# monkey0head/RePlay_cql

Measured on AMD Instinct MI355X. Metric: CQL train-steps/sec, higher is better.
Workload: dtype bf16; 1 GPU; BASELINE.json configs[2]: synthetic 1000000 users x 100000 items, CQL d=128, L=50, B=4096/GPU, bf16 MFMA + fp32 accumulate; users=1000000, items=100000, d=128, window=50, batch_per_gpu=4096, global_batch=4096, parallelism=dp1 (users sharded by rank, RCCL gradient all-reduce), k=10, dp_variant=single

## Files before the change

replay_cql_amd/csrc/common.h:

```cpp
#pragma once
#include <hip/hip_runtime.h>
#include <stdint.h>
#include <stdio.h>
#include <stdarg.h>

#include "../../include/cqlrec.h"

typedef __attribute__((ext_vector_type(8))) __bf16 bf16x8;
typedef __attribute__((ext_vector_type(4))) __bf16 bf16x4;
typedef __attribute__((ext_vector_type(16))) float f32x16;
typedef __attribute__((ext_vector_type(4))) float f32x4;
typedef __attribute__((address_space(3))) bf16x4 lds_bf16x4;

#define CQL_WAVE 64
#define CQL_LOG2E 1.4426950408889634f
#define CQL_LN2 0.6931471805599453f
#define NEG_INF_F (-__builtin_inff())

void cql_set_error(const char* fmt, ...);
#define CQL_REQUIRE(cond, ...)            \
  do {                                    \
    if (!(cond)) {                        \
      cql_set_error(__VA_ARGS__);         \
      return CQLREC_ERR_INVALID;          \
// ... 59 lines not shown
}

__device__ __forceinline__ int mfma_row(int reg, int half) { return (reg & 3) + 8 * (reg >> 2) + 4 * half; }

template <int D>
__device__ __forceinline__ int swz_chunk(int row, int ch) {
  if constexpr (D == 64) return ch ^ ((row >> 1) & 7);
  else return ch ^ (row & 15);
}

__device__ __forceinline__ float fast_exp2(float x) { return __builtin_amdgcn_exp2f(x); }

__device__ __forceinline__ uint32_t f32_order_key(float f) {
  uint32_t u = __float_as_uint(f);
  return (u & 0x80000000u) ? ~u : (u | 0x80000000u);
}
__device__ __forceinline__ float f32_from_order_key(uint32_t k) {
  uint32_t u = (k & 0x80000000u) ? (k & 0x7FFFFFFFu) : ~k;
  return __uint_as_float(u);
}

struct CqlAdamFix {
  int valid;
  const float* slab;
  const float* slab_cs;
  int32_t G, T, nblk, items, D;
  float scale;
  int64_t n_items;
  int64_t rows_off, cs_off;
};
int cql_adam_ema_fix(float* theta, float* grads, float* m, float* v, float* target, uint16_t* theta_b, uint16_t* target_b,
                     int64_t n, float step_size, float sqrt_bc2, float beta1, float beta2, float eps, float tau,
                     int32_t zero_grads, const CqlAdamFix* fix, hipStream_t stream);
int cql_adam_ema_rows(float* theta, float* grads, float* m, float* v, float* target, uint16_t* theta_b, uint16_t* target_b,
                      int64_t n, float step_size, float sqrt_bc2, float beta1, float beta2, float eps, float tau,
                      int32_t zero_grads, const uint8_t* row_map, int32_t d, int64_t n_rows, hipStream_t stream);
int cql_gather_pool_bwd_mark_rows(const void* ws, int64_t n_states, int32_t L, int32_t d, int64_t n_items, uint8_t* row_map,
                                  hipStream_t s);
```

replay_cql_amd/csrc/gbwd.hip:

```cpp
#include <cstring>
#include <rocprim/device/device_radix_sort.hpp>

#include "common.h"

__global__ __launch_bounds__(256) void gbwd_pairs_kernel(const int64_t* __restrict__ offsets,
                                                         const int32_t* __restrict__ items,
                                                         const int32_t* __restrict__ users,
                                                         const int32_t* __restrict__ ends, int end_delta,
                                                         int64_t n_states, int L, uint32_t pad_key,
                                                         uint32_t* __restrict__ keys, uint32_t* __restrict__ vals,
                                                         int32_t* __restrict__ lens) {
  const int lane = threadIdx.x & 63;
  const int64_t state = (int64_t)blockIdx.x * 4 + (threadIdx.x >> 6);
  if (state >= n_states) return;
  const int u = users[state];
  const int64_t o0 = offsets[u];
  const int end = ends ? (ends[state] + end_delta) : (int)(offsets[u + 1] - o0);
  const int len = end < L ? end : L;
  if (lane == 0) lens[state] = len;
  const int32_t* win = items + o0 + end - len;
  for (int j = lane; j < L; j += 64) {
    keys[state * L + j] = (j < len) ? (uint32_t)win[j] : pad_key;
    vals[state * L + j] = (uint32_t)state;
  }
// ... 200 lines not shown
  if (e != hipSuccess) {
    cql_set_error("gather_pool_bwd_prepare: radix sort failed: %s", hipGetErrorString(e));
    return CQLREC_ERR_HIP;
  }
  CQL_LAUNCH_CHECK("gather_pool_bwd_prepare");
  return CQLREC_OK;
}

__global__ __launch_bounds__(256) void gbwd_mark_rows_kernel(const uint32_t* __restrict__ keys, int64_t n_pairs,
                                                             uint32_t pad_key, uint8_t* __restrict__ row_map) {
  const int64_t i = (int64_t)blockIdx.x * blockDim.x + threadIdx.x;
  if (i >= n_pairs) return;
  const uint32_t k = keys[i];
  if (k < pad_key) row_map[k] = 1;
}
int cql_gather_pool_bwd_mark_rows(const void* ws, int64_t n_states, int32_t L, int32_t d, int64_t n_items, uint8_t* row_map,
                                  hipStream_t s) {
  CQL_REQUIRE(ws && row_map, "gather_pool_bwd_mark_rows: NULL pointer");
  CQL_REQUIRE(n_items > 0 && n_items < (1ll << 31), "gather_pool_bwd_mark_rows: n_items=%lld", (long long)n_items);
  if (hipMemsetAsync(row_map, 0, (size_t)n_items, s) != hipSuccess) {
    cql_set_error("gather_pool_bwd_mark_rows: clearing the map failed");
    return CQLREC_ERR_HIP;
  }
  if (n_states <= 0) return CQLREC_OK;
  const GbWs w = gb_carve(const_cast<void*>(ws), n_states, L, d);
  const int64_t n = n_states * L;
  CqlProfScope prof(CQLREC_PH_GATHER_BWD, s);
  hipLaunchKernelGGL(gbwd_mark_rows_kernel, dim3(cql_ceil_div(n, 256)), dim3(256), 0, s, w.keys_out, n, (uint32_t)n_items,
                     row_map);
  CQL_LAUNCH_CHECK("gather_pool_bwd_mark_rows");
  return CQLREC_OK;
}

extern "C" int cqlrec_gather_pool_bwd_apply(const float* dh0, int64_t n_states, int32_t L, int32_t d, int64_t n_items,
                                            void* ws, int64_t ws_bytes, float* g_E_in, cqlrec_stream stream) {
  CQL_REQUIRE(dh0 && ws && g_E_in, "gather_pool_bwd_apply: NULL pointer");
  CQL_REQUIRE(d == 64 || d == 128 || d == 256, "gather_pool_bwd_apply: d=%d unsupported", d);
  if (n_states <= 0) return CQLREC_OK;
  CQL_REQUIRE(ws_bytes >= cqlrec_gather_pool_bwd_ws_bytes(n_states, L, d), "gather_pool_bwd_apply: workspace too small");
  const GbWs w = gb_carve(ws, n_states, L, d);
  const int64_t n = n_states * L;
  hipStream_t s = (hipStream_t)stream;
  const uint32_t pad_key = (uint32_t)n_items;
  CqlProfScope prof(CQLREC_PH_GATHER_BWD, s);
  const int64_t n4 = n_states * (d / 4);
  hipLaunchKernelGGL(gbwd_scale_kernel, dim3(cql_ceil_div(n4, 256)), dim3(256), 0, s, (const float4*)dh0, w.lens, n4,
                     d / 4, (float4*)w.g);
  segsum_launch<false, GB_CH>(w.g, nullptr, w.keys_out, w.vals_out, n, pad_key, d, g_E_in, nullptr, w.edge, nullptr, s);
  CQL_LAUNCH_CHECK("gather_pool_bwd_apply");
  return CQLREC_OK;
}

extern "C" int cqlrec_gather_pool_bwd_sorted(const float* dh0, const int64_t* offsets, const int32_t* items,
                                             const int32_t* users, const int32_t* ends, int32_t end_delta,
                                             int64_t n_states, int32_t L, int32_t d, int64_t n_items, void* ws,
                                             int64_t ws_bytes, float* g_E_in, cqlrec_stream stream) {
  int rc = cqlrec_gather_pool_bwd_prepare(offsets, items, users, ends, end_delta, n_states, L, d, n_items, ws, ws_bytes,
                                          stream);
  if (rc != CQLREC_OK) return rc;
  return cqlrec_gather_pool_bwd_apply(dh0, n_states, L, d, n_items, ws, ws_bytes, g_E_in, stream);
}


namespace {
struct OhWs {
  uint32_t *keys_in, *vals_in, *keys_out, *vals_out;
// ... 65 lines not shown
```

replay_cql_amd/csrc/misc.hip:

```cpp
#include <stdlib.h>
#include "common.h"
#include "adam_math.h"

static thread_local char g_err[512] = "";
void cql_set_error(const char* fmt, ...) {
  va_list ap;
  va_start(ap, fmt);
  vsnprintf(g_err, sizeof(g_err), fmt, ap);
  va_end(ap);
}
extern "C" const char* cqlrec_last_error(void) { return g_err; }
extern "C" int cqlrec_abi_version(void) { return CQLREC_ABI_VERSION; }

#define CQL_PROF_POOL 8192
static struct {
  bool on = false;
  bool created = false;
  hipEvent_t ev[CQL_PROF_POOL][2];
  int phase[CQL_PROF_POOL];
  int n = 0;
  int open = -1;
  uint32_t mask = 0xFFFFFFFFu;
} g_prof;

// ... 661 lines not shown
  CQL_LAUNCH_CHECK("td_loss");
  return CQLREC_OK;
}

template <bool NT>
__global__ __launch_bounds__(256) void adam_ema_kernel(float4* __restrict__ theta, float4* __restrict__ grads,
                                                       float4* __restrict__ m, float4* __restrict__ v,
                                                       float4* __restrict__ target, uint2* __restrict__ theta_b,
                                                       uint2* __restrict__ target_b, int64_t n4, float step_size,
                                                       float sqrt_bc2, float beta1, float beta2, float eps, float tau,
                                                       int zero_grads) {
  const float omb1 = 1.0f - beta1, omb2 = 1.0f - beta2, omt = 1.0f - tau;
  for (int64_t i = (int64_t)blockIdx.x * blockDim.x + threadIdx.x; i < n4; i += (int64_t)gridDim.x * blockDim.x) {
    const float4 g4 = ld4<NT>(grads + i);
    float4 p4 = ld4<NT>(theta + i), m4 = ld4<NT>(m + i), v4 = ld4<NT>(v + i), t4 = ld4<NT>(target + i);
    const float g[4] = {g4.x, g4.y, g4.z, g4.w};
    float p[4] = {p4.x, p4.y, p4.z, p4.w}, mm[4] = {m4.x, m4.y, m4.z, m4.w}, vv[4] = {v4.x, v4.y, v4.z, v4.w},
          tt[4] = {t4.x, t4.y, t4.z, t4.w};
#pragma unroll
    for (int k = 0; k < 4; ++k) {
      adam_ema_elem(g[k], p[k], mm[k], vv[k], tt[k], step_size, sqrt_bc2, beta1, beta2, eps, tau, omb1, omb2, omt);
    }
    st4<NT>(theta + i, p[0], p[1], p[2], p[3]);
    st4<NT>(m + i, mm[0], mm[1], mm[2], mm[3]);
    st4<NT>(v + i, vv[0], vv[1], vv[2], vv[3]);
    st4<NT>(target + i, tt[0], tt[1], tt[2], tt[3]);
    theta_b[i] = make_uint2(pack_bf16x2(p[0], p[1]), pack_bf16x2(p[2], p[3]));
    target_b[i] = make_uint2(pack_bf16x2(tt[0], tt[1]), pack_bf16x2(tt[2], tt[3]));
    if (zero_grads) st4<NT>(grads + i, 0.f, 0.f, 0.f, 0.f);
  }
}

template <bool NT>
__global__ __launch_bounds__(256) void adam_ema_rows_kernel(float4* __restrict__ theta, float4* __restrict__ grads,
                                                            float4* __restrict__ m, float4* __restrict__ v,
                                                            float4* __restrict__ target, uint2* __restrict__ theta_b,
                                                            uint2* __restrict__ target_b, int64_t n4, float step_size,
                                                            float sqrt_bc2, float beta1, float beta2, float eps, float tau,
                                                            int zero_grads, const uint8_t* __restrict__ row_map, int ld4row,
                                                            int64_t n_rows) {
  const float omb1 = 1.0f - beta1, omb2 = 1.0f - beta2, omt = 1.0f - tau;
  for (int64_t i = (int64_t)blockIdx.x * blockDim.x + threadIdx.x; i < n4; i += (int64_t)gridDim.x * blockDim.x) {
    const int64_t row = i >> ld4row;
    const bool live = row < n_rows && row_map[row] != 0;
    float4 p4 = ld4<NT>(theta + i), m4 = ld4<NT>(m + i), v4 = ld4<NT>(v + i), t4 = ld4<NT>(target + i);
    float4 g4 = make_float4(0.f, 0.f, 0.f, 0.f);
    if (live) g4 = ld4<NT>(grads + i);
    const float g[4] = {g4.x, g4.y, g4.z, g4.w};
    float p[4] = {p4.x, p4.y, p4.z, p4.w}, mm[4] = {m4.x, m4.y, m4.z, m4.w}, vv[4] = {v4.x, v4.y, v4.z, v4.w},
          tt[4] = {t4.x, t4.y, t4.z, t4.w};
#pragma unroll
    for (int k = 0; k < 4; ++k) {
      adam_ema_elem(g[k], p[k], mm[k], vv[k], tt[k], step_size, sqrt_bc2, beta1, beta2, eps, tau, omb1, omb2, omt);
    }
    st4<NT>(theta + i, p[0], p[1], p[2], p[3]);
    st4<NT>(m + i, mm[0], mm[1], mm[2], mm[3]);
    st4<NT>(v + i, vv[0], vv[1], vv[2], vv[3]);
    st4<NT>(target + i, tt[0], tt[1], tt[2], tt[3]);
    theta_b[i] = make_uint2(pack_bf16x2(p[0], p[1]), pack_bf16x2(p[2], p[3]));
    target_b[i] = make_uint2(pack_bf16x2(tt[0], tt[1]), pack_bf16x2(tt[2], tt[3]));
    if (zero_grads) st4<NT>(grads + i, 0.f, 0.f, 0.f, 0.f);
  }
}

int cql_adam_ema_rows(float* theta, float* grads, float* m, float* v, float* target, uint16_t* theta_b, uint16_t* target_b,
                      int64_t n, float step_size, float sqrt_bc2, float beta1, float beta2, float eps, float tau,
                      int32_t zero_grads, const uint8_t* row_map, int32_t d, int64_t n_rows, hipStream_t stream) {
  CQL_REQUIRE(theta && grads && m && v && target && theta_b && target_b && row_map, "adam_ema_rows: NULL pointer");
  CQL_REQUIRE(n > 0 && n % 4 == 0, "adam_ema_rows: n=%lld must be a positive multiple of 4", (long long)n);
  CQL_REQUIRE(d == 64 || d == 128 || d == 256, "adam_ema_rows: d=%d unsupported", d);
  CQL_REQUIRE(n_rows >= 0 && n_rows * d <= n, "adam_ema_rows: %lld rows of %d do not fit n=%lld", (long long)n_rows, d,
              (long long)n);
  const int64_t n4 = n / 4;
  int blocks = (int)((n4 + 255) / 256);
  if (blocks > 8192) blocks = 8192;
  CqlProfScope prof(CQLREC_PH_ADAM, stream);
  hipLaunchKernelGGL(adam_ema_rows_kernel<true>, dim3(blocks), dim3(256), 0, stream, (float4*)theta, (float4*)grads,
                     (float4*)m, (float4*)v, (float4*)target, (uint2*)theta_b, (uint2*)target_b, n4, step_size, sqrt_bc2,
                     beta1, beta2, eps, tau, zero_grads, row_map, __builtin_ctz((unsigned)d) - 2, n_rows);
  CQL_LAUNCH_CHECK("adam_ema (row map)");
  return CQLREC_OK;
}

__device__ __forceinline__ void adam_fix4(const CqlAdamFix& f, float (&g)[4], int64_t i4, int ld, int li) {
  const int64_t e = 4 * i4;
  uint32_t item;
  int col = -1;
  if (e >= f.rows_off && e < f.rows_off + f.n_items * f.D) {
    const uint64_t r = (uint64_t)(e - f.rows_off);
    item = (uint32_t)(r >> ld);
    col = (int)(r & (uint64_t)(f.D - 1));
  } else if (e >= f.cs_off && e < f.cs_off + f.n_items) {
    item = (uint32_t)(e - f.cs_off);
  } else {
    return;
  }
#ifdef ADAMFIX_ABL_NOLOOP
  return;
#endif
  const uint32_t grp = item >> li, row = item & (uint32_t)(f.items - 1);
  const uint32_t W = (uint32_t)f.G * (uint32_t)f.T, nblk = (uint32_t)f.nblk, lo = grp * (uint32_t)f.T, hi = lo + (uint32_t)f.T;
  for (uint32_t p = ((lo + 1) * nblk + W - 1) / W; p < nblk; ++p) {
    const uint32_t u0 = (uint32_t)((uint64_t)p * W / nblk);
    if (u0 >= hi) break;
    if (u0 <= lo) continue;
    if ((uint32_t)(((uint64_t)p + 1) * W / nblk) == u0) continue;
    if (col >= 0) {
      const float4 s4 = *reinterpret_cast<const float4*>(f.slab + ((int64_t)p * f.items + row) * f.D + col);
      g[0] += f.scale * s4.x; g[1] += f.scale * s4.y; g[2] += f.scale * s4.z; g[3] += f.scale * s4.w;
    } else {
      const float* sc = f.slab_cs + (int64_t)p * f.items + row;
#pragma unroll
      for (int k = 0; k < 4; ++k)
// ... 93 lines not shown
```

replay_cql_amd/csrc/train.hip:

```cpp
#include <math.h>
#include <stdlib.h>
#include "common.h"
#include "qhead_internal.h"

static int g_concurrency = -1;

enum { MK_LOSS = 0, MK_DH, MK_DE, MK_CHAIN, MK_ADAM_IN, MK_ADAM_OUT, MK_PROLOGUE, MK_LSE, MK_NEXT_LOSS, MK_ENC_DX, MK_GATHER_BWD, MK_SORT_NEXT, MK_COUNT };
static hipEvent_t g_marks[MK_COUNT];
static int g_marks_on = 0;
static int g_mark_phase = 0;
static void mark(int k, hipStream_t s) {
  if (g_marks_on && g_mark_phase) (void)hipEventRecord(g_marks[k], s);
}
extern "C" int cqlrec_debug_marks_enable(int32_t on) {
  if (on && !g_marks[0])
    for (int i = 0; i < MK_COUNT; ++i)
      if (hipEventCreate(&g_marks[i]) != hipSuccess) return CQLREC_ERR_HIP;
  g_marks_on = on ? 1 : 0;
  return CQLREC_OK;
}
extern "C" int cqlrec_debug_marks_read(float* ms_out) {
  if (!g_marks[0] || !ms_out) return CQLREC_ERR_INVALID;
  for (int i = 0; i < MK_COUNT; ++i) {
    ms_out[i] = -1.f;
    if (hipEventSynchronize(g_marks[i]) != hipSuccess) continue;
    float ms = 0.f;
    if (hipEventElapsedTime(&ms, g_marks[MK_LOSS], g_marks[i]) == hipSuccess) ms_out[i] = ms;
  }
  return CQLREC_OK;
}

namespace {
struct Carve {
  char* base;
  int64_t off;
  explicit Carve(void* p) : base((char*)p), off(0) {}
  template <typename T>
  T* take(int64_t n) {
    T* p = base ? (T*)(base + off) : nullptr;
    off += (n * (int64_t)sizeof(T) + 255) / 256 * 256;
    return p;
  }
};

struct StepWs {
  int32_t *users, *tpos, *act, *a_star;
  float *rew, *done, *q_a, *lse, *nlse2, *nlse_nat, *q_targ, *y, *coef, *maxv, *loss, *term;
  float *h0_s, *dH, *dh0;
  uint16_t *h0b, *zb, *hb, *h0b_t, *zb_t, *hb_t;
  void *ws_q, *ws_q2, *ws_qb, *ws_qb2, *ws_enc, *ws_gb, *ws_oh;
  uint8_t* row_map;
  int64_t ws_q_bytes, ws_qb_bytes, ws_qf_bytes, ws_enc_bytes, ws_gb_bytes, ws_oh_bytes;
  int64_t total;
};

void carve_small(Carve& c, StepWs& w, int32_t B, int32_t d) {
  w.users = c.take<int32_t>(B);
  w.tpos = c.take<int32_t>(B);
  w.act = c.take<int32_t>(B);
  w.a_star = c.take<int32_t>(B);
  w.rew = c.take<float>(B);
  w.done = c.take<float>(B);
  w.q_a = c.take<float>(B);
  w.lse = c.take<float>(B);
  w.nlse2 = c.take<float>(B);
  w.nlse_nat = c.take<float>(B);
  w.q_targ = c.take<float>(B);
  w.y = c.take<float>(B);
  w.coef = c.take<float>(B);
  w.maxv = c.take<float>(B);
  w.loss = c.take<float>(64);
  w.term = c.take<float>(B);
  w.h0_s = c.take<float>((int64_t)B * d);
  w.dH = c.take<float>((int64_t)B * d);
  w.dh0 = c.take<float>((int64_t)B * d);
  w.h0b = c.take<uint16_t>((int64_t)2 * B * d);
  w.zb = c.take<uint16_t>((int64_t)2 * B * d);
  w.hb = c.take<uint16_t>((int64_t)2 * B * d);
  w.h0b_t = c.take<uint16_t>((int64_t)B * d);
  w.zb_t = c.take<uint16_t>((int64_t)B * d);
  w.hb_t = c.take<uint16_t>((int64_t)B * d);
}

StepWs carve_step(void* ws, int32_t B, int64_t N, int32_t d, int32_t L, uint64_t step = 0) {
  StepWs w, other;
  Carve c(ws);
  if (step & 1) {
    carve_small(c, other, B, d);
    carve_small(c, w, B, d);
  } else {
    carve_small(c, w, B, d);
    carve_small(c, other, B, d);
  }
  w.ws_q_bytes = cqlrec_qhead_ws_bytes(B, N, d);
  w.ws_q = c.take<char>(w.ws_q_bytes);
  w.ws_q2 = c.take<char>(w.ws_q_bytes);
  w.ws_qb_bytes = cqlrec_qhead_bwd_ws_bytes(B, N, d);
  w.ws_qf_bytes = w.ws_qb_bytes + w.ws_q_bytes;
  w.ws_qb = c.take<char>(w.ws_qf_bytes);
  w.ws_qb2 = c.take<char>(w.ws_qb_bytes);
  w.ws_enc_bytes = cqlrec_encoder_bwd_ws_bytes(B, d);
  w.ws_enc = c.take<char>(w.ws_enc_bytes);
  w.ws_gb_bytes = cqlrec_gather_pool_bwd_ws_bytes(B, L, d);
  void* gb0 = c.take<char>(w.ws_gb_bytes);
  void* gb1 = c.take<char>(w.ws_gb_bytes);
  w.ws_gb = (step & 1) ? gb1 : gb0;
  w.ws_oh_bytes = cql_onehot_ws_bytes(B, d);
  void* oh0 = c.take<char>(w.ws_oh_bytes);
  void* oh1 = c.take<char>(w.ws_oh_bytes);
  w.ws_oh = (step & 1) ? oh1 : oh0;
  uint8_t* rm0 = c.take<uint8_t>(N);
  uint8_t* rm1 = c.take<uint8_t>(N);
  w.row_map = (step & 1) ? rm1 : rm0;
  w.total = c.off;
  return w;
}

int check_ctx(const cqlrec_train_ctx* c) {
  CQL_REQUIRE(c != nullptr, "train_step: ctx is NULL");
  CQL_REQUIRE(c->offsets && c->items && c->rewards, "train_step: CSR pointers are NULL");
  CQL_REQUIRE(c->theta && c->grads && c->adam_m && c->adam_v && c->target && c->theta_b && c->target_b,
              "train_step: model state pointers are NULL");
  CQL_REQUIRE(c->ws != nullptr, "train_step: workspace is NULL");
  CQL_REQUIRE(c->batch > 0 && c->window > 0 && c->world > 0 && c->rank >= 0 && c->rank < c->world,
              "train_step: batch=%d window=%d world=%d rank=%d", c->batch, c->window, c->world, c->rank);
  const int32_t d = c->layout.d;
  CQL_REQUIRE(d == 64 || d == 128 || d == 256, "train_step: d=%d unsupported", d);
  CQL_REQUIRE(c->ws_bytes >= cqlrec_train_ws_bytes(c->batch, c->layout.n_items, d, c->window),
              "train_step: workspace too small");
  return CQLREC_OK;
}
}

extern "C" int cqlrec_set_concurrency(int32_t on) {
  g_concurrency = on ? 1 : 0;
  return CQLREC_OK;
}

extern "C" int64_t cqlrec_train_ws_bytes(int32_t batch, int64_t n_items, int32_t d, int32_t window) {
  return carve_step(nullptr, batch, n_items, d, window).total + 256;
}

#define CQL_TRY(expr)            \
  do {                           \
    int rc__ = (expr);           \
    if (rc__ != CQLREC_OK) return rc__; \
  } while (0)

namespace {
struct SideStream {
  hipStream_t s = nullptr;
  hipStream_t s2 = nullptr;
  hipStream_t s3 = nullptr;
  hipEvent_t sorted[2] = {nullptr, nullptr};
  hipEvent_t forked = nullptr, fork2 = nullptr, join2 = nullptr;
  hipEvent_t loss = nullptr, items = nullptr, dh = nullptr, eout = nullptr, presample = nullptr, fwd_done = nullptr;
  bool ok = false;
  bool tried = false;
};
bool concurrency_on() {
  if (g_concurrency < 0) {
    const char* v = getenv("CQL_CONCURRENCY");
    g_concurrency = (v && *v == '0') ? 0 : 1;
  }
  return g_concurrency != 0;
}
__global__ __launch_bounds__(64) void cql_pipe_hog_kernel(int spins) {
  extern __shared__ volatile char pad[];
  pad[threadIdx.x] = 1;
  for (int i = 0; i < spins; ++i) __builtin_amdgcn_s_sleep(127);
  pad[threadIdx.x + 64] = pad[threadIdx.x];
}
__global__ void cql_pipe_tiny_kernel() {}

struct PipeProbe {
  hipEvent_t a0 = nullptr, a1 = nullptr, b1 = nullptr;
  bool ok = false;
  PipeProbe() {
    ok = hipEventCreate(&a0) == hipSuccess && hipEventCreate(&a1) == hipSuccess && hipEventCreate(&b1) == hipSuccess;
  }
  ~PipeProbe() {
    if (a0) (void)hipEventDestroy(a0);
    if (a1) (void)hipEventDestroy(a1);
    if (b1) (void)hipEventDestroy(b1);
  }
  int conflict(hipStream_t x, hipStream_t y) {
    if (!ok || hipDeviceSynchronize() != hipSuccess) return -1;
    (void)hipEventRecord(a0, x);
    hipLaunchKernelGGL(cql_pipe_hog_kernel, dim3(8192), dim3(64), 60 * 1024, x, 3);
// ... 55 lines not shown
  if (!*extra && hipStreamCreateWithFlags(extra, hipStreamNonBlocking) != hipSuccess) return false;
  return hipDeviceSynchronize() == hipSuccess;
}

SideStream& side_stream() {
  static SideStream per_device[CQL_MAX_DEVICES];
  static SideStream off;
  if (!concurrency_on()) return off;
  const int slot = cql_device_slot();
  SideStream& ss = per_device[slot];
  if (!ss.tried) {
    ss.tried = true;
    hipStream_t pk[3] = {};
    hipStream_t extra = nullptr;
    ss.ok = pick_streams(nullptr, pk, &extra, &g_pick_report[slot]);
    if (ss.ok) {
      ss.s2 = pk[0];
      ss.s = pk[1];
      ss.s3 = pk[2];
      if (!g_aux[slot][0]) g_aux[slot][0] = pk[2];
      if (!g_aux[slot][1]) g_aux[slot][1] = extra;
    }
    ss.ok = ss.ok &&
            hipEventCreateWithFlags(&ss.sorted[0], hipEventDisableTiming) == hipSuccess &&
            hipEventCreateWithFlags(&ss.sorted[1], hipEventDisableTiming) == hipSuccess &&
            hipEventCreateWithFlags(&ss.forked, hipEventDisableTiming) == hipSuccess &&
            hipEventCreateWithFlags(&ss.fork2, hipEventDisableTiming) == hipSuccess &&
            hipEventCreateWithFlags(&ss.join2, hipEventDisableTiming) == hipSuccess &&
            hipEventCreateWithFlags(&ss.loss, hipEventDisableTiming) == hipSuccess &&
            hipEventCreateWithFlags(&ss.items, hipEventDisableTiming) == hipSuccess &&
            hipEventCreateWithFlags(&ss.dh, hipEventDisableTiming) == hipSuccess &&
            hipEventCreateWithFlags(&ss.eout, hipEventDisableTiming) == hipSuccess &&
            hipEventCreateWithFlags(&ss.presample, hipEventDisableTiming) == hipSuccess &&
            hipEventCreateWithFlags(&ss.fwd_done, hipEventDisableTiming) == hipSuccess;
  }
  return ss;
}

bool need_side_streams(SideStream& ss, bool want_s3 = false) {
  (void)want_s3;
  return ss.ok;
}

struct StepPtrs {
  const uint16_t *Ein_b, *Eout_b, *W1_b, *W2_b, *tEin_b, *tEout_b, *tW1_b, *tW2_b;
  const float *b_out, *b1, *b2, *tb_out, *tb1, *tb2;
};
float alpha_scale(const cqlrec_train_ctx* c) { return (float)(c->alpha / ((double)c->batch * (double)c->world)); }
StepPtrs step_ptrs(const cqlrec_train_ctx* c) {
  const cqlrec_layout& L = c->layout;
  StepPtrs p;
  p.Ein_b = c->theta_b + L.off_E_in;   p.Eout_b = c->theta_b + L.off_E_out;
  p.W1_b = c->theta_b + L.off_W1;      p.W2_b = c->theta_b + L.off_W2;
  p.b_out = c->theta + L.off_b_out;    p.b1 = c->theta + L.off_b1;   p.b2 = c->theta + L.off_b2;
  p.tEin_b = c->target_b + L.off_E_in; p.tEout_b = c->target_b + L.off_E_out;
  p.tW1_b = c->target_b + L.off_W1;    p.tW2_b = c->target_b + L.off_W2;
  p.tb_out = c->target + L.off_b_out;  p.tb1 = c->target + L.off_b1; p.tb2 = c->target + L.off_b2;
  return p;
}
}

extern "C" int cqlrec_runtime_init(void) {
  int dev = -1;
  if (hipGetDevice(&dev) != hipSuccess || dev < 0) {
    cql_set_error("runtime_init: no HIP device");
    return CQLREC_ERR_HIP;
// ... 1 lines not shown
  const int slot = cql_device_slot();
  if (concurrency_on()) {
    if (!side_stream().ok) {
      cql_set_error("runtime_init: creating the internal streams failed");
      return CQLREC_ERR_HIP;
    }
  } else {
    for (int i = 0; i < CQLREC_AUX_STREAMS; ++i)
      if (!g_aux[slot][i] && hipStreamCreateWithFlags(&g_aux[slot][i], hipStreamNonBlocking) != hipSuccess) {
        cql_set_error("runtime_init: creating aux stream %d failed", i);
        return CQLREC_ERR_HIP;
      }
  }
  return CQLREC_OK;
}

extern "C" int cqlrec_runtime_probe_count(void) { return g_pick_report[cql_device_slot()]; }

extern "C" cqlrec_stream cqlrec_aux_stream(int32_t index) {
  if (index < 0 || index >= CQLREC_AUX_STREAMS) return nullptr;
  return (cqlrec_stream)g_aux[cql_device_slot()][index];
}


#define CQL_HIP_TRY(expr, what)                 \
  do {                                          \
    if ((expr) != hipSuccess) {                 \
      cql_set_error("%s: %s failed", what, #expr); \
      return CQLREC_ERR_HIP;                    \
    }                                           \
  } while (0)

namespace {
int sample_ahead(const cqlrec_train_ctx* c, uint64_t step, cqlrec_stream stream, hipEvent_t sampled_ev) {
  const cqlrec_layout& L = c->layout;
  StepWs w = carve_step(c->ws, c->batch, L.n_items, L.d, c->window, step);
  CQL_TRY(cqlrec_sample_transitions(c->offsets, c->items, c->rewards, c->n_users, c->seed, step,
                                    (uint64_t)c->rank * (uint64_t)c->batch, c->batch, w.users, w.tpos, w.act, w.rew,
                                    w.done, stream));
  CQL_HIP_TRY(hipEventRecord(sampled_ev, (hipStream_t)stream), "train_steps");
  CQL_TRY(cqlrec_gather_pool_bwd_prepare(c->offsets, c->items, w.users, w.tpos, 0, c->batch, c->window, L.d, L.n_items,
                                         w.ws_gb, w.ws_gb_bytes, stream));
  CQL_TRY(cql_gather_pool_bwd_mark_rows(w.ws_gb, c->batch, c->window, L.d, L.n_items, w.row_map, (hipStream_t)stream));
  return cql_onehot_prepare(w.act, c->batch, L.n_items, L.d, w.ws_oh, w.ws_oh_bytes, (hipStream_t)stream);
}

int backward_items_long_impl(const cqlrec_train_ctx* c, uint64_t step, cqlrec_stream stream, CqlAdamFix* fix);
int loss_sum_impl(const cqlrec_train_ctx* c, uint64_t step, float* loss_out, hipStream_t on) {
  StepWs w = carve_step(c->ws, c->batch, c->layout.n_items, c->layout.d, c->window, step);
  const float inv_batch = 1.0f / ((float)c->batch * (float)c->world);
  return cql_td_loss_sum(w.term, c->batch, inv_batch, loss_out ? loss_out : w.loss, on);
}
int forward_impl(const cqlrec_train_ctx* c, uint64_t step, float* loss_out, cqlrec_stream stream, hipEvent_t eout_ready,
                 hipEvent_t presampled = nullptr, hipStream_t early_items = nullptr, CqlAdamFix* early_fix = nullptr,
                 bool* loss_sum_deferred = nullptr, bool want_row_map = false) {
  const cqlrec_layout& L = c->layout;
  const int32_t B = c->batch, d = L.d, W = c->window;
  const int64_t N = L.n_items;
  StepWs w = carve_step(c->ws, B, N, d, W, step);
  const StepPtrs p = step_ptrs(c);
  const int64_t Bd = (int64_t)B * d;
  hipStream_t s = (hipStream_t)stream;

  SideStream& ss = side_stream();
  if (presampled) {
    CQL_HIP_TRY(hipStreamWaitEvent(s, presampled, 0), "train_step_forward");
  } else {
    CQL_TRY(cqlrec_sample_transitions(c->offsets, c->items, c->rewards, c->n_users, c->seed, step,
                                      (uint64_t)c->rank * (uint64_t)B, B, w.users, w.tpos, w.act, w.rew, w.done, stream));
    if (ss.ok && need_side_streams(ss)) {
      if (hipEventRecord(ss.forked, s) != hipSuccess || hipStreamWaitEvent(ss.s, ss.forked, 0) != hipSuccess) ss.ok = false;
    }
  }
// ... 150 lines not shown
extern "C" int cqlrec_train_step_backward_items(const cqlrec_train_ctx* c, uint64_t step, cqlrec_stream stream) {
  CQL_TRY(check_ctx(c));
  if (g_early_long[step & 1]) {
    g_early_long[step & 1] = false;
    const cqlrec_layout& L = c->layout;
    CQL_TRY(backward_items_onehot_impl(c, step, stream));
    return cql_qde_fixup_deferred(g_early_fix[step & 1], c->grads + L.off_E_out, c->grads + L.off_b_out, (hipStream_t)stream);
  }
  return backward_items_impl(c, step, stream);
}

extern "C" int cqlrec_train_step_backward_rest(const cqlrec_train_ctx* c, uint64_t step, cqlrec_stream stream) {
  CQL_TRY(check_ctx(c));
  return backward_rest_impl(c, step, stream);
}

extern "C" int cqlrec_train_step_fwd_bwd(const cqlrec_train_ctx* c, uint64_t step, float* loss_out,
                                         cqlrec_stream stream) {
  CQL_TRY(cqlrec_train_step_forward(c, step, loss_out, stream));
  SideStream& ss = side_stream();
  hipStream_t s = (hipStream_t)stream;
  if (need_side_streams(ss) && hipEventRecord(ss.loss, s) == hipSuccess && hipStreamWaitEvent(ss.s, ss.loss, 0) == hipSuccess) {
    CQL_TRY(backward_items_impl(c, step, (cqlrec_stream)ss.s));
    CQL_HIP_TRY(hipEventRecord(ss.items, ss.s), "train_step_fwd_bwd");
    CQL_TRY(backward_rest_impl(c, step, stream));
    CQL_HIP_TRY(hipStreamWaitEvent(s, ss.items, 0), "train_step_fwd_bwd");
    return CQLREC_OK;
  }
  CQL_TRY(backward_rest_impl(c, step, stream));
  return backward_items_impl(c, step, stream);
}

int update_range_impl(const cqlrec_train_ctx* c, uint64_t step, int64_t lo, int64_t hi, cqlrec_stream stream,
                      const CqlAdamFix* fix, int zero_grads = 1, const uint8_t* row_map = nullptr);
extern "C" int cqlrec_train_steps(const cqlrec_train_ctx* c, uint64_t step0, int32_t n_steps, float* loss_out,
                                  cqlrec_stream stream) {
  CQL_TRY(check_ctx(c));
  CQL_REQUIRE(n_steps >= 0, "train_steps: n_steps=%d", n_steps);
  CQL_REQUIRE(c->world == 1, "train_steps: world=%d; data-parallel callers use the phase entry points", c->world);
  const cqlrec_layout& L = c->layout;
  hipStream_t s = (hipStream_t)stream;
  hipEvent_t pending = nullptr;
  hipEvent_t sampled = nullptr;
  need_side_streams(side_stream(), true);
  const bool use_map = n_steps > 1 && L.off_E_in == 0;
  bool grads_dirty = false;
  for (int32_t i = 0; i < n_steps; ++i) {
    const uint64_t step = step0 + (uint64_t)i;
    const bool lean = use_map && i + 1 < n_steps;
    static const int early_de = !(getenv("CQL_EARLY_DE") && getenv("CQL_EARLY_DE")[0] == '0');
    SideStream& ss0 = side_stream();
    const bool early = early_de && ss0.ok && ss0.s;
    CqlAdamFix fix = {};
    bool sum_deferred = false;
    const bool can_defer = ss0.ok && ss0.s3 && i + 1 < n_steps;
    CQL_TRY(forward_impl(c, step, loss_out ? loss_out + i : nullptr, stream, pending, sampled, early ? ss0.s : nullptr, &fix,
                         can_defer ? &sum_deferred : nullptr, use_map));
    pending = sampled = nullptr;
    if (g_marks_on && n_steps >= 4) {
      if (i == n_steps / 2) g_mark_phase = 1;
      else if (i == n_steps / 2 + 1) g_mark_phase = 0;
    }
    SideStream& ss = side_stream();
    if (g_mark_phase == 1) mark(MK_LOSS, s);
    if (ss.ok && hipEventRecord(ss.loss, s) == hipSuccess) {
      if (i + 1 < n_steps && hipStreamWaitEvent(ss.s3, ss.loss, 0) == hipSuccess) {
        if (sum_deferred) {
          CQL_TRY(loss_sum_impl(c, step, loss_out ? loss_out + i : nullptr, ss.s3));
          sum_deferred = false;
        }
        CQL_TRY(sample_ahead(c, step + 1, (cqlrec_stream)ss.s3, ss.presample));
        CQL_HIP_TRY(hipEventRecord(ss.sorted[(step + 1) & 1], ss.s3), "train_steps");
        if (g_mark_phase == 1) mark(MK_SORT_NEXT, ss.s3);
        sampled = ss.presample;
      }
      if (sum_deferred) CQL_TRY(loss_sum_impl(c, step, loss_out ? loss_out + i : nullptr, s));
      CQL_HIP_TRY(hipStreamWaitEvent(ss.s, ss.loss, 0), "train_steps");
      if (early)
        CQL_TRY(backward_items_onehot_impl(c, step, (cqlrec_stream)ss.s));
      else
        CQL_TRY(backward_items_impl(c, step, (cqlrec_stream)ss.s, &fix));
      if (g_mark_phase == 1) mark(MK_DE, ss.s);
      CQL_TRY(backward_states_impl(c, step, stream));
      if (g_mark_phase == 1) mark(MK_DH, s);
      CQL_TRY(backward_chain_impl(c, step, stream));
      if (g_mark_phase == 1) mark(MK_CHAIN, s);
      CQL_TRY(cqlrec_train_step_update_range(c, step, L.off_W1, L.total, stream));
      if (use_map) {
        const StepWs w = carve_step(c->ws, c->batch, L.n_items, L.d, c->window, step);
        CQL_TRY(update_range_impl(c, step, 0, L.off_E_out, stream, nullptr, lean ? 0 : 1, w.row_map));
      } else {
        CQL_TRY(cqlrec_train_step_update_range(c, step, 0, L.off_E_out, stream));
      }
      if (g_mark_phase == 1) mark(MK_ADAM_IN, s);
      CQL_HIP_TRY(hipStreamWaitEvent(ss.s, ss.dh, 0), "train_steps");
      fix.rows_off = 0;
      fix.cs_off = L.off_b_out - L.off_E_out;
      CQL_TRY(update_range_impl(c, step, L.off_E_out, L.off_W1, (cqlrec_stream)ss.s, &fix, lean ? 0 : 1));
      grads_dirty = lean;
      CQL_HIP_TRY(hipEventRecord(ss.eout, ss.s), "train_steps");
      if (g_mark_phase == 1) { mark(MK_ADAM_OUT, ss.s); g_mark_phase = 2; }
      pending = ss.eout;
    } else {
      CQL_REQUIRE(!grads_dirty, "train_steps: lost the side streams in the middle of a call");
      if (sum_deferred) CQL_TRY(loss_sum_impl(c, step, loss_out ? loss_out + i : nullptr, s));
      CQL_TRY(backward_rest_impl(c, step, stream));
      CQL_TRY(backward_items_impl(c, step, stream));
      CQL_TRY(cqlrec_train_step_update_range(c, step, 0, L.total, stream));
    }
  }
  g_mark_phase = 0;
  if (pending) CQL_HIP_TRY(hipStreamWaitEvent(s, pending, 0), "train_steps");
  return CQLREC_OK;
}

extern "C" int cqlrec_train_step_update_range(const cqlrec_train_ctx* c, uint64_t step, int64_t lo, int64_t hi,
                                              cqlrec_stream stream) {
  return update_range_impl(c, step, lo, hi, stream, nullptr);
}

int update_range_impl(const cqlrec_train_ctx* c, uint64_t step, int64_t lo, int64_t hi, cqlrec_stream stream,
                      const CqlAdamFix* fix, int zero_grads, const uint8_t* row_map) {
  CQL_TRY(check_ctx(c));
  CQL_REQUIRE(lo >= 0 && hi <= c->layout.total && lo < hi && lo % 4 == 0 && hi % 4 == 0,
              "train_step_update_range: bad range [%lld, %lld)", (long long)lo, (long long)hi);
  const double t = (double)(step + 1);
  const double bc1 = 1.0 - pow((double)c->beta1, t);
  const double bc2 = 1.0 - pow((double)c->beta2, t);
  const float step_size = (float)((double)c->lr / bc1);
  const float sqrt_bc2 = (float)sqrt(bc2);
  if (row_map) {
    CQL_REQUIRE(lo == c->layout.off_E_in && !fix, "train_step_update_range: the row map belongs to the E_in range");
    return cql_adam_ema_rows(c->theta + lo, c->grads + lo, c->adam_m + lo, c->adam_v + lo, c->target + lo, c->theta_b + lo,
                             c->target_b + lo, hi - lo, step_size, sqrt_bc2, (float)c->beta1, (float)c->beta2, (float)c->eps,
                             (float)c->tau, zero_grads, row_map, c->layout.d, c->layout.n_items, (hipStream_t)stream);
  }
  return cql_adam_ema_fix(c->theta + lo, c->grads + lo, c->adam_m + lo, c->adam_v + lo, c->target + lo, c->theta_b + lo,
                          c->target_b + lo, hi - lo, step_size, sqrt_bc2, (float)c->beta1, (float)c->beta2, (float)c->eps,
                          (float)c->tau, zero_grads, fix, (hipStream_t)stream);
}

extern "C" int cqlrec_train_step_update(const cqlrec_train_ctx* c, uint64_t step, cqlrec_stream stream) {
  CQL_TRY(check_ctx(c));
  return cqlrec_train_step_update_range(c, step, 0, c->layout.total, stream);
}

extern "C" int cqlrec_train_views_get(const cqlrec_train_ctx* c, uint64_t step, cqlrec_train_views* out) {
  CQL_TRY(check_ctx(c));
  CQL_REQUIRE(out != nullptr, "train_views_get: out is NULL");
  const int32_t B = c->batch, d = c->layout.d;
  StepWs w = carve_step(c->ws, B, c->layout.n_items, d, c->window, step);
  out->users = w.users; out->tpos = w.tpos; out->act = w.act; out->a_star = w.a_star;
  out->rew = w.rew; out->done = w.done; out->q_a = w.q_a; out->lse = w.lse; out->q_targ = w.q_targ;
  out->y = w.y; out->coef = w.coef; out->dH = w.dH; out->dh0 = w.dh0; out->h0_s = w.h0_s;
  out->hb_s = w.hb; out->hb_sn = w.hb + (int64_t)B * d; out->hb_tn = w.hb_t;
  return CQLREC_OK;
}
```

Baseline: 1487 train-steps/s (B=4096 transitions per step and GPU).

## Defer Adam updates for E_in rows not read by the next step

Adds a per-step read map of the item rows the next batch will gather, plus a per-row age counter. The E_in Adam/EMA kernel now skips rows that have no gradient and will not be read next step, and replays the missed zero-gradient steps in a loop when the row is next touched. A host table holds the per-step bias-correction scalars. This is meant to cut the full-table pass over 100k x 128 fp32 theta, m, v and target on most steps. The cost is an extra marking kernel and memset, a stream wait on the read-map event, and variable per-thread work when stale rows catch up (at most 64 steps).

```diff
diff --git a/replay_cql_amd/csrc/common.h b/replay_cql_amd/csrc/common.h
--- a/replay_cql_amd/csrc/common.h
+++ b/replay_cql_amd/csrc/common.h
@@ -115,8 +115,15 @@
 int cql_adam_ema_fix(float* theta, float* grads, float* m, float* v, float* target, uint16_t* theta_b, uint16_t* target_b,
                      int64_t n, float step_size, float sqrt_bc2, float beta1, float beta2, float eps, float tau,
                      int32_t zero_grads, const CqlAdamFix* fix, hipStream_t stream);
-int cql_adam_ema_rows(float* theta, float* grads, float* m, float* v, float* target, uint16_t* theta_b, uint16_t* target_b,
-                      int64_t n, float step_size, float sqrt_bc2, float beta1, float beta2, float eps, float tau,
-                      int32_t zero_grads, const uint8_t* row_map, int32_t d, int64_t n_rows, hipStream_t stream);
+#define CQL_ADAM_DEFER_CAP 64
+struct CqlAdamSteps {
+  float step_size[CQL_ADAM_DEFER_CAP], sqrt_bc2[CQL_ADAM_DEFER_CAP];
+};
+int cql_adam_ema_rows_deferred(float* theta, float* grads, float* m, float* v, float* target, uint16_t* theta_b,
+                               uint16_t* target_b, int64_t n, const CqlAdamSteps& tab, uint64_t step, float beta1, float beta2,
+                               float eps, float tau, int32_t zero_grads, const uint8_t* row_map, const uint8_t* read_next,
+                               uint8_t* age, int32_t d, int64_t n_rows, hipStream_t stream);
+int cql_mark_read_rows(const int64_t* offsets, const int32_t* items, const int32_t* users, const int32_t* tpos,
+                       int64_t n_states, int32_t L, int64_t n_items, uint8_t* read_map, hipStream_t s);
 int cql_gather_pool_bwd_mark_rows(const void* ws, int64_t n_states, int32_t L, int32_t d, int64_t n_items, uint8_t* row_map,
                                   hipStream_t s);
diff --git a/replay_cql_amd/csrc/gbwd.hip b/replay_cql_amd/csrc/gbwd.hip
--- a/replay_cql_amd/csrc/gbwd.hip
+++ b/replay_cql_amd/csrc/gbwd.hip
@@ -256,6 +256,36 @@
   return CQLREC_OK;
 }
 
+__global__ __launch_bounds__(256) void mark_read_rows_kernel(const int64_t* __restrict__ offsets,
+                                                             const int32_t* __restrict__ items,
+                                                             const int32_t* __restrict__ users,
+                                                             const int32_t* __restrict__ tpos, int64_t n_states, int L,
+                                                             uint32_t n_items, uint8_t* __restrict__ read_map) {
+  const int64_t t = (int64_t)blockIdx.x * blockDim.x + threadIdx.x;
+  const int64_t b = t / (L + 1);
+  const int j = (int)(t % (L + 1));
+  if (b >= n_states) return;
+  const int tp = tpos[b];
+  if (j > (tp < L ? tp : L)) return;
+  const uint32_t it = (uint32_t)items[offsets[users[b]] + tp - j];
+  if (it < n_items) read_map[it] = 1;
+}
+int cql_mark_read_rows(const int64_t* offsets, const int32_t* items, const int32_t* users, const int32_t* tpos,
+                       int64_t n_states, int32_t L, int64_t n_items, uint8_t* read_map, hipStream_t s) {
+  CQL_REQUIRE(offsets && items && users && tpos && read_map, "mark_read_rows: NULL pointer");
+  CQL_REQUIRE(n_items > 0 && n_items < (1ll << 31) && L > 0, "mark_read_rows: n_items=%lld L=%d", (long long)n_items, L);
+  if (hipMemsetAsync(read_map, 0, (size_t)n_items, s) != hipSuccess) {
+    cql_set_error("mark_read_rows: clearing the map failed");
+    return CQLREC_ERR_HIP;
+  }
+  if (n_states <= 0) return CQLREC_OK;
+  CqlProfScope prof(CQLREC_PH_GATHER_BWD, s);
+  hipLaunchKernelGGL(mark_read_rows_kernel, dim3(cql_ceil_div(n_states * (L + 1), 256)), dim3(256), 0, s, offsets, items,
+                     users, tpos, n_states, L, (uint32_t)n_items, read_map);
+  CQL_LAUNCH_CHECK("mark_read_rows");
+  return CQLREC_OK;
+}
+
 extern "C" int cqlrec_gather_pool_bwd_apply(const float* dh0, int64_t n_states, int32_t L, int32_t d, int64_t n_items,
                                             void* ws, int64_t ws_bytes, float* g_E_in, cqlrec_stream stream) {
   CQL_REQUIRE(dh0 && ws && g_E_in, "gather_pool_bwd_apply: NULL pointer");
diff --git a/replay_cql_amd/csrc/misc.hip b/replay_cql_amd/csrc/misc.hip
--- a/replay_cql_amd/csrc/misc.hip
+++ b/replay_cql_amd/csrc/misc.hip
@@ -717,53 +717,73 @@
 }
 
 template <bool NT>
-__global__ __launch_bounds__(256) void adam_ema_rows_kernel(float4* __restrict__ theta, float4* __restrict__ grads,
-                                                            float4* __restrict__ m, float4* __restrict__ v,
-                                                            float4* __restrict__ target, uint2* __restrict__ theta_b,
-                                                            uint2* __restrict__ target_b, int64_t n4, float step_size,
-                                                            float sqrt_bc2, float beta1, float beta2, float eps, float tau,
-                                                            int zero_grads, const uint8_t* __restrict__ row_map, int ld4row,
-                                                            int64_t n_rows) {
+__global__ __launch_bounds__(256) void adam_ema_rows_deferred_kernel(
+    float4* __restrict__ theta, float4* __restrict__ grads, float4* __restrict__ m, float4* __restrict__ v,
+    float4* __restrict__ target, uint2* __restrict__ theta_b, uint2* __restrict__ target_b, int64_t n4, CqlAdamSteps tab,
+    uint32_t step, float beta1, float beta2, float eps, float tau, int zero_grads, const uint8_t* __restrict__ row_map,
+    const uint8_t* __restrict__ read_next, uint8_t* age, int ld4row, int64_t n_rows) {
+  __shared__ float2 tab_s[CQL_ADAM_DEFER_CAP];
+  if (threadIdx.x < CQL_ADAM_DEFER_CAP)
+    tab_s[threadIdx.x] = make_float2(tab.step_size[threadIdx.x], tab.sqrt_bc2[threadIdx.x]);
+  __syncthreads();
   const float omb1 = 1.0f - beta1, omb2 = 1.0f - beta2, omt = 1.0f - tau;
+  float zero = 0.f;
+  asm volatile("" : "+v"(zero));
+  const int64_t row_lane = ((int64_t)1 << ld4row) - 1;
   for (int64_t i = (int64_t)blockIdx.x * blockDim.x + threadIdx.x; i < n4; i += (int64_t)gridDim.x * blockDim.x) {
     const int64_t row = i >> ld4row;
-    const bool live = row < n_rows && row_map[row] != 0;
-    float4 p4 = ld4<NT>(theta + i), m4 = ld4<NT>(m + i), v4 = ld4<NT>(v + i), t4 = ld4<NT>(target + i);
-    float4 g4 = make_float4(0.f, 0.f, 0.f, 0.f);
-    if (live) g4 = ld4<NT>(grads + i);
-    const float g[4] = {g4.x, g4.y, g4.z, g4.w};
-    float p[4] = {p4.x, p4.y, p4.z, p4.w}, mm[4] = {m4.x, m4.y, m4.z, m4.w}, vv[4] = {v4.x, v4.y, v4.z, v4.w},
-          tt[4] = {t4.x, t4.y, t4.z, t4.w};
-#pragma unroll
-    for (int k = 0; k < 4; ++k) {
-      adam_ema_elem(g[k], p[k], mm[k], vv[k], tt[k], step_size, sqrt_bc2, beta1, beta2, eps, tau, omb1, omb2, omt);
-    }
-    st4<NT>(theta + i, p[0], p[1], p[2], p[3]);
-    st4<NT>(m + i, mm[0], mm[1], mm[2], mm[3]);
-    st4<NT>(v + i, vv[0], vv[1], vv[2], vv[3]);
-    st4<NT>(target + i, tt[0], tt[1], tt[2], tt[3]);
-    theta_b[i] = make_uint2(pack_bf16x2(p[0], p[1]), pack_bf16x2(p[2], p[3]));
-    target_b[i] = make_uint2(pack_bf16x2(tt[0], tt[1]), pack_bf16x2(tt[2], tt[3]));
+    bool live = false, go = true;
+    int k = 1;
+    if (row < n_rows) {
+      live = row_map[row] != 0;
+      k = (int)age[row] + 1;
+      go = live || !read_next || read_next[row] != 0 || k >= CQL_ADAM_DEFER_CAP;
+      if ((i & row_lane) == 0) age[row] = go ? (uint8_t)0 : (uint8_t)k;
+    }
+    if (go) {
+      float4 p4 = ld4<NT>(theta + i), m4 = ld4<NT>(m + i), v4 = ld4<NT>(v + i), t4 = ld4<NT>(target + i);
+      float4 g4 = make_float4(zero, zero, zero, zero);
+      if (live) g4 = ld4<NT>(grads + i);
+      const float gc[4] = {g4.x, g4.y, g4.z, g4.w};
+      float p[4] = {p4.x, p4.y, p4.z, p4.w}, mm[4] = {m4.x, m4.y, m4.z, m4.w}, vv[4] = {v4.x, v4.y, v4.z, v4.w},
+            tt[4] = {t4.x, t4.y, t4.z, t4.w};
+      for (int a = k - 1; a >= 0; --a) {
+        const float2 sc = tab_s[(step - (uint32_t)a) & (uint32_t)(CQL_ADAM_DEFER_CAP - 1)];
+#pragma unroll
+        for (int j = 0; j < 4; ++j) {
+          const float g = a == 0 ? gc[j] : zero;
+          adam_ema_elem(g, p[j], mm[j], vv[j], tt[j], sc.x, sc.y, beta1, beta2, eps, tau, omb1, omb2, omt);
+        }
+      }
+      st4<NT>(theta + i, p[0], p[1], p[2], p[3]);
+      st4<NT>(m + i, mm[0], mm[1], mm[2], mm[3]);
+      st4<NT>(v + i, vv[0], vv[1], vv[2], vv[3]);
+      st4<NT>(target + i, tt[0], tt[1], tt[2], tt[3]);
+      theta_b[i] = make_uint2(pack_bf16x2(p[0], p[1]), pack_bf16x2(p[2], p[3]));
+      target_b[i] = make_uint2(pack_bf16x2(tt[0], tt[1]), pack_bf16x2(tt[2], tt[3]));
+    }
     if (zero_grads) st4<NT>(grads + i, 0.f, 0.f, 0.f, 0.f);
   }
 }
 
-int cql_adam_ema_rows(float* theta, float* grads, float* m, float* v, float* target, uint16_t* theta_b, uint16_t* target_b,
-                      int64_t n, float step_size, float sqrt_bc2, float beta1, float beta2, float eps, float tau,
-                      int32_t zero_grads, const uint8_t* row_map, int32_t d, int64_t n_rows, hipStream_t stream) {
-  CQL_REQUIRE(theta && grads && m && v && target && theta_b && target_b && row_map, "adam_ema_rows: NULL pointer");
-  CQL_REQUIRE(n > 0 && n % 4 == 0, "adam_ema_rows: n=%lld must be a positive multiple of 4", (long long)n);
-  CQL_REQUIRE(d == 64 || d == 128 || d == 256, "adam_ema_rows: d=%d unsupported", d);
-  CQL_REQUIRE(n_rows >= 0 && n_rows * d <= n, "adam_ema_rows: %lld rows of %d do not fit n=%lld", (long long)n_rows, d,
-              (long long)n);
+int cql_adam_ema_rows_deferred(float* theta, float* grads, float* m, float* v, float* target, uint16_t* theta_b,
+                               uint16_t* target_b, int64_t n, const CqlAdamSteps& tab, uint64_t step, float beta1, float beta2,
+                               float eps, float tau, int32_t zero_grads, const uint8_t* row_map, const uint8_t* read_next,
+                               uint8_t* age, int32_t d, int64_t n_rows, hipStream_t stream) {
+  CQL_REQUIRE(theta && grads && m && v && target && theta_b && target_b && row_map && age,
+              "adam_ema_rows_deferred: NULL pointer");
+  CQL_REQUIRE(n > 0 && n % 4 == 0, "adam_ema_rows_deferred: n=%lld must be a positive multiple of 4", (long long)n);
+  CQL_REQUIRE(d == 64 || d == 128 || d == 256, "adam_ema_rows_deferred: d=%d unsupported", d);
+  CQL_REQUIRE(n_rows >= 0 && n_rows * d <= n, "adam_ema_rows_deferred: %lld rows of %d do not fit n=%lld", (long long)n_rows,
+              d, (long long)n);
   const int64_t n4 = n / 4;
   int blocks = (int)((n4 + 255) / 256);
   if (blocks > 8192) blocks = 8192;
   CqlProfScope prof(CQLREC_PH_ADAM, stream);
-  hipLaunchKernelGGL(adam_ema_rows_kernel<true>, dim3(blocks), dim3(256), 0, stream, (float4*)theta, (float4*)grads,
-                     (float4*)m, (float4*)v, (float4*)target, (uint2*)theta_b, (uint2*)target_b, n4, step_size, sqrt_bc2,
-                     beta1, beta2, eps, tau, zero_grads, row_map, __builtin_ctz((unsigned)d) - 2, n_rows);
-  CQL_LAUNCH_CHECK("adam_ema (row map)");
+  hipLaunchKernelGGL(adam_ema_rows_deferred_kernel<true>, dim3(blocks), dim3(256), 0, stream, (float4*)theta, (float4*)grads,
+                     (float4*)m, (float4*)v, (float4*)target, (uint2*)theta_b, (uint2*)target_b, n4, tab, (uint32_t)step,
+                     beta1, beta2, eps, tau, zero_grads, row_map, read_next, age, __builtin_ctz((unsigned)d) - 2, n_rows);
+  CQL_LAUNCH_CHECK("adam_ema (deferred rows)");
   return CQLREC_OK;
 }
 
diff --git a/replay_cql_amd/csrc/train.hip b/replay_cql_amd/csrc/train.hip
--- a/replay_cql_amd/csrc/train.hip
+++ b/replay_cql_amd/csrc/train.hip
@@ -50,6 +50,8 @@
   uint16_t *h0b, *zb, *hb, *h0b_t, *zb_t, *hb_t;
   void *ws_q, *ws_q2, *ws_qb, *ws_qb2, *ws_enc, *ws_gb, *ws_oh;
   uint8_t* row_map;
+  uint8_t* read_map;
+  uint8_t* age;
   int64_t ws_q_bytes, ws_qb_bytes, ws_qf_bytes, ws_enc_bytes, ws_gb_bytes, ws_oh_bytes;
   int64_t total;
 };
@@ -112,6 +114,10 @@
   uint8_t* rm0 = c.take<uint8_t>(N);
   uint8_t* rm1 = c.take<uint8_t>(N);
   w.row_map = (step & 1) ? rm1 : rm0;
+  uint8_t* rd0 = c.take<uint8_t>(N);
+  uint8_t* rd1 = c.take<uint8_t>(N);
+  w.read_map = (step & 1) ? rd1 : rd0;
+  w.age = c.take<uint8_t>(N);
   w.total = c.off;
   return w;
 }
@@ -155,6 +161,7 @@
   hipEvent_t sorted[2] = {nullptr, nullptr};
   hipEvent_t forked = nullptr, fork2 = nullptr, join2 = nullptr;
   hipEvent_t loss = nullptr, items = nullptr, dh = nullptr, eout = nullptr, presample = nullptr, fwd_done = nullptr;
+  hipEvent_t read_map = nullptr;
   bool ok = false;
   bool tried = false;
 };
@@ -276,6 +283,7 @@
             hipEventCreateWithFlags(&ss.dh, hipEventDisableTiming) == hipSuccess &&
             hipEventCreateWithFlags(&ss.eout, hipEventDisableTiming) == hipSuccess &&
             hipEventCreateWithFlags(&ss.presample, hipEventDisableTiming) == hipSuccess &&
+            hipEventCreateWithFlags(&ss.read_map, hipEventDisableTiming) == hipSuccess &&
             hipEventCreateWithFlags(&ss.fwd_done, hipEventDisableTiming) == hipSuccess;
   }
   return ss;
@@ -343,13 +351,17 @@
   } while (0)
 
 namespace {
-int sample_ahead(const cqlrec_train_ctx* c, uint64_t step, cqlrec_stream stream, hipEvent_t sampled_ev) {
+int sample_ahead(const cqlrec_train_ctx* c, uint64_t step, cqlrec_stream stream, hipEvent_t sampled_ev,
+                 hipEvent_t read_map_ev) {
   const cqlrec_layout& L = c->layout;
   StepWs w = carve_step(c->ws, c->batch, L.n_items, L.d, c->window, step);
   CQL_TRY(cqlrec_sample_transitions(c->offsets, c->items, c->rewards, c->n_users, c->seed, step,
                                     (uint64_t)c->rank * (uint64_t)c->batch, c->batch, w.users, w.tpos, w.act, w.rew,
                                     w.done, stream));
   CQL_HIP_TRY(hipEventRecord(sampled_ev, (hipStream_t)stream), "train_steps");
+  CQL_TRY(cql_mark_read_rows(c->offsets, c->items, w.users, w.tpos, c->batch, c->window, L.n_items, w.read_map,
+                             (hipStream_t)stream));
+  CQL_HIP_TRY(hipEventRecord(read_map_ev, (hipStream_t)stream), "train_steps");
   CQL_TRY(cqlrec_gather_pool_bwd_prepare(c->offsets, c->items, w.users, w.tpos, 0, c->batch, c->window, L.d, L.n_items,
                                          w.ws_gb, w.ws_gb_bytes, stream));
   CQL_TRY(cql_gather_pool_bwd_mark_rows(w.ws_gb, c->batch, c->window, L.d, L.n_items, w.row_map, (hipStream_t)stream));
@@ -566,7 +578,16 @@
 }
 
 int update_range_impl(const cqlrec_train_ctx* c, uint64_t step, int64_t lo, int64_t hi, cqlrec_stream stream,
-                      const CqlAdamFix* fix, int zero_grads = 1, const uint8_t* row_map = nullptr);
+                      const CqlAdamFix* fix, int zero_grads = 1);
+namespace {
+void adam_step_scalars(const cqlrec_train_ctx* c, uint64_t step, float* step_size, float* sqrt_bc2) {
+  const double t = (double)(step + 1);
+  const double bc1 = 1.0 - pow((double)c->beta1, t);
+  const double bc2 = 1.0 - pow((double)c->beta2, t);
+  *step_size = (float)((double)c->lr / bc1);
+  *sqrt_bc2 = (float)sqrt(bc2);
+}
+}
 extern "C" int cqlrec_train_steps(const cqlrec_train_ctx* c, uint64_t step0, int32_t n_steps, float* loss_out,
                                   cqlrec_stream stream) {
   CQL_TRY(check_ctx(c));
@@ -578,6 +599,11 @@
   hipEvent_t sampled = nullptr;
   need_side_streams(side_stream(), true);
   const bool use_map = n_steps > 1 && L.off_E_in == 0;
+  CqlAdamSteps adam_tab = {};
+  if (use_map) {
+    const StepWs w0 = carve_step(c->ws, c->batch, L.n_items, L.d, c->window, step0);
+    CQL_HIP_TRY(hipMemsetAsync(w0.age, 0, (size_t)L.n_items, s), "train_steps");
+  }
   bool grads_dirty = false;
   for (int32_t i = 0; i < n_steps; ++i) {
     const uint64_t step = step0 + (uint64_t)i;
@@ -603,7 +629,7 @@
           CQL_TRY(loss_sum_impl(c, step, loss_out ? loss_out + i : nullptr, ss.s3));
           sum_deferred = false;
         }
-        CQL_TRY(sample_ahead(c, step + 1, (cqlrec_stream)ss.s3, ss.presample));
+        CQL_TRY(sample_ahead(c, step + 1, (cqlrec_stream)ss.s3, ss.presample, ss.read_map));
         CQL_HIP_TRY(hipEventRecord(ss.sorted[(step + 1) & 1], ss.s3), "train_steps");
         if (g_mark_phase == 1) mark(MK_SORT_NEXT, ss.s3);
         sampled = ss.presample;
@@ -622,7 +648,16 @@
       CQL_TRY(cqlrec_train_step_update_range(c, step, L.off_W1, L.total, stream));
       if (use_map) {
         const StepWs w = carve_step(c->ws, c->batch, L.n_items, L.d, c->window, step);
-        CQL_TRY(update_range_impl(c, step, 0, L.off_E_out, stream, nullptr, lean ? 0 : 1, w.row_map));
+        const int slot = (int)(step % CQL_ADAM_DEFER_CAP);
+        adam_step_scalars(c, step, &adam_tab.step_size[slot], &adam_tab.sqrt_bc2[slot]);
+        const uint8_t* read_next = nullptr;
+        if (lean && sampled) {
+          CQL_HIP_TRY(hipStreamWaitEvent(s, ss.read_map, 0), "train_steps");
+          read_next = carve_step(c->ws, c->batch, L.n_items, L.d, c->window, step + 1).read_map;
+        }
+        CQL_TRY(cql_adam_ema_rows_deferred(c->theta, c->grads, c->adam_m, c->adam_v, c->target, c->theta_b, c->target_b,
+                                           L.off_E_out, adam_tab, step, (float)c->beta1, (float)c->beta2, (float)c->eps,
+                                           (float)c->tau, lean ? 0 : 1, w.row_map, read_next, w.age, L.d, L.n_items, s));
       } else {
         CQL_TRY(cqlrec_train_step_update_range(c, step, 0, L.off_E_out, stream));
       }
@@ -654,21 +689,12 @@
 }
 
 int update_range_impl(const cqlrec_train_ctx* c, uint64_t step, int64_t lo, int64_t hi, cqlrec_stream stream,
-                      const CqlAdamFix* fix, int zero_grads, const uint8_t* row_map) {
+                      const CqlAdamFix* fix, int zero_grads) {
   CQL_TRY(check_ctx(c));
   CQL_REQUIRE(lo >= 0 && hi <= c->layout.total && lo < hi && lo % 4 == 0 && hi % 4 == 0,
               "train_step_update_range: bad range [%lld, %lld)", (long long)lo, (long long)hi);
-  const double t = (double)(step + 1);
-  const double bc1 = 1.0 - pow((double)c->beta1, t);
-  const double bc2 = 1.0 - pow((double)c->beta2, t);
-  const float step_size = (float)((double)c->lr / bc1);
-  const float sqrt_bc2 = (float)sqrt(bc2);
-  if (row_map) {
-    CQL_REQUIRE(lo == c->layout.off_E_in && !fix, "train_step_update_range: the row map belongs to the E_in range");
-    return cql_adam_ema_rows(c->theta + lo, c->grads + lo, c->adam_m + lo, c->adam_v + lo, c->target + lo, c->theta_b + lo,
-                             c->target_b + lo, hi - lo, step_size, sqrt_bc2, (float)c->beta1, (float)c->beta2, (float)c->eps,
-                             (float)c->tau, zero_grads, row_map, c->layout.d, c->layout.n_items, (hipStream_t)stream);
-  }
+  float step_size, sqrt_bc2;
+  adam_step_scalars(c, step, &step_size, &sqrt_bc2);
   return cql_adam_ema_fix(c->theta + lo, c->grads + lo, c->adam_m + lo, c->adam_v + lo, c->target + lo, c->theta_b + lo,
                           c->target_b + lo, hi - lo, step_size, sqrt_bc2, (float)c->beta1, (float)c->beta2, (float)c->eps,
                           (float)c->tau, zero_grads, fix, (hipStream_t)stream);
```

New measurement: 1536 train-steps/s (B=4096 transitions per step and GPU), median of 6. 3.3% higher.
